# mrvollger/rustybam

Hardware: AMD Instinct MI355X
Metric: CIGAR-ops/s, liftover over 100 kb sliding windows (whole pass, inputs resident in HBM) (higher is better)
Workload: dtype u32

## Files before the change

### rustybam_amd/csrc/capi.hip

```cpp
#include <hip/hip_runtime.h>
#include <sys/mman.h>

#include <algorithm>
#include <cstdarg>
#include <cstdio>
#include <cstdlib>
#include <cstring>
#include <ctime>
#include <numeric>
#include <string>
#include <thread>
#include <vector>
#include <chrono>
#include <map>
#include <mutex>

#include "../../include/rustybam_amd.h"
#include "rb_lift.h"
#include "rb_trim.h"
#include "rb_launch.h"

#ifndef RB_SCAN_ROWS_MEAN_MAX
#define RB_SCAN_ROWS_MEAN_MAX 1536
#endif
// ... 676 lines not shown
    int rc = RB_OK;
    std::vector<uint32_t> slot_of(n_rec);
    for (uint64_t w = 0; w < n_rec; w++) slot_of[sched[w]] = (uint32_t)w;
    if (!rc) rc = upload_vec(ctx, sched, &pl->sched);
    if (!rc) rc = upload_vec(ctx, slot_of, &pl->slot_of);
    if (!rc) rc = upload_vec(ctx, ident, &pl->ident);
    if (!rc) rc = upload_vec(ctx, canon_pos, &pl->canon_pos);
    if (!rc) rc = upload_vec(ctx, g_st, &pl->w_st);
    if (!rc) rc = upload_vec(ctx, g_en, &pl->w_en);
    if (!rc) rc = upload_vec(ctx, g_orig, &pl->w_orig);
    if (!rc) rc = upload_vec(ctx, o_st, &pl->wo_st);
    if (!rc) rc = upload_vec(ctx, o_en, &pl->wo_en);
    if (!rc) rc = upload_vec(ctx, cw_off, &pl->cw_off);
    if (!rc) rc = upload_vec(ctx, mono, &pl->cw_mono);
    if (!rc && pl->n_tiles) rc = upload_vec(ctx, tiles, &pl->tiles);
    if (!rc && hipStreamSynchronize(ctx->stream) != hipSuccess) rc = fail(ctx, RB_E_HIP, "plan upload: %s", hipGetErrorString(hipGetLastError()));
    if (rc) {
        rb_plan_destroy(pl);
        return rc;
    }
    *out = pl;
    return RB_OK;
}
extern "C" void rb_plan_destroy(rb_plan *pl) {
    if (!pl) return;
    void *ptrs[] = {pl->sched, pl->slot_of, pl->ident, pl->canon_pos, pl->w_st, pl->w_en, pl->w_orig, pl->wo_st, pl->wo_en, pl->cw_off, pl->cw_mono, pl->tiles};
    for (void *q : ptrs)
        if (q) (void)rb_dev_free(pl->ctx, q);
    delete pl;
}

struct ws_layout {
    size_t hit_off, win_lo, block_sums, arena, pend_count, pend_list, jobs, gen_list, x_st, x_en, bp_tmp, bp_off, bp_cur, brk_rows, copy_count, copy_list, decl_count, decl_list, gen_cp, diag_stamps, fb_count, fb_list, starts_bad, total;
};
static bool rb_no_gen_cp() {
    static const bool v = getenv("RB_DEBUG_NO_GEN_CP") != nullptr;
    return v;
}
static ws_layout ws_of(uint64_t n_rec, uint64_t rows_cap, uint64_t n_ops) {
    ws_layout w;
    size_t o = 0;
    auto take = [&](size_t bytes) {
        size_t at = o;
        o += (bytes + 255) & ~(size_t)255;
        return at;
    };
    w.hit_off = take((n_rec + 2) * 8);
    w.win_lo = take((n_rec + 2) * 4);
    w.block_sums = take(rb_scan_block_sums_count(n_rec) * 8);
    w.arena = take((size_t)RB_MAX_ARENA * RB_ARENA_STRIDE * 8);
    w.pend_count = take(256);
    w.pend_list = take((n_rec + 1) * 4);
    w.jobs = take((n_rec + 1) * sizeof(rb_job));
    w.gen_list = take((rows_cap + 1) * 4);
    w.x_st = take((rows_cap + 1) * 8);
    w.x_en = take((rows_cap + 1) * 8);
    w.bp_tmp = take((rows_cap + 1) * 8);
    w.bp_off = take((n_rec + 1) * 8);
    w.bp_cur = take((size_t)RB_MAX_ARENA * 128);
    w.brk_rows = take((rows_cap + 1) * sizeof(rb_hit_row));
    w.copy_count = take(256);
    w.copy_list = take((rows_cap + 1) * 16);
    w.decl_count = take(256);
    w.decl_list = take((n_rec + 1) * 4);
    w.gen_cp = take(rb_no_gen_cp() ? 256 : (size_t)(n_ops / RB_GCP + n_rec + 2) * sizeof(uint4));
    w.diag_stamps = take((n_rec + 1) * 4);
    w.fb_count = take(256);
    w.fb_list = take((n_rec + 1) * 4);
    w.starts_bad = take(256);
    w.total = o;
    return w;
}
extern "C" size_t rb_plan_workspace_bytes(const rb_plan *plan, uint64_t rows_cap) {
    if (!plan) return 0;
    return ws_of(plan->n_rec, rows_cap, plan->n_ops).total;
}
extern "C" size_t rb_plan_diag_stamps_offset(const rb_plan *plan, uint64_t rows_cap) {
    if (!plan) return 0;
    return ws_of(plan->n_rec, rows_cap, plan->n_ops).diag_stamps;
}

static uint64_t slot_stride_of(uint64_t n_ops, uint64_t n_rec) { return ((n_ops + 31) & ~(uint64_t)31) + 32 * n_rec + 64; }
extern "C" uint64_t rb_plan_out_capacity(const rb_plan *plan, int for_break) {
    if (!plan) return 0;
    const uint64_t slots = for_break ? std::min<uint32_t>(2u, RB_MS) : std::min<uint32_t>(plan->depth, RB_MS);
    return slots * slot_stride_of(plan->n_ops, plan->n_rec) + plan->n_ops / 16 + 32 * plan->n_rec + (1u << 20);
}

static uint32_t pick_arenas(uint64_t n_rec) {
    uint64_t a = n_rec / 256;
    if (a < 1) a = 1;
    if (a > RB_MAX_ARENA) a = RB_MAX_ARENA;
    return (uint32_t)a;
}

static int lift_common(rb_ctx *ctx, const rb_plan *plan, const rb_batch_view *b, const rb_norm_row *norm, int policy,
                       void *workspace, rb_hit_row *rows, uint64_t rows_cap, uint32_t *out_ops, uint64_t out_cap,
                       rb_counters *counters, bool is_break, uint32_t max_size) {
    if (!ctx || !plan || !b || !norm || !workspace || !counters) return RB_E_INVALID;
    if (b->n_rec != plan->n_rec) return fail(ctx, RB_E_INVALID, "plan was built for %llu records, batch has %llu", (unsigned long long)plan->n_rec, (unsigned long long)b->n_rec);
// ... 51 lines not shown
    p.fused = (policy & RB_LIFT_FUSED_SCAN) ? 1 : 0;
    p.op_starts = (policy & RB_LIFT_OP_STARTS) ? 1 : 0;
    if (p.op_starts && p.fused) return fail(ctx, RB_E_INVALID, "RB_LIFT_OP_STARTS takes finished norm_rows: not together with RB_LIFT_FUSED_SCAN");
    if (p.op_starts && (policy & RB_LIFT_DESCRIPTORS)) return fail(ctx, RB_E_INVALID, "RB_LIFT_OP_STARTS with RB_LIFT_DESCRIPTORS: a descriptor indexes the record's ORIGINAL cigar, which a batch cut in place no longer is");
    if (p.op_starts && b->n_ops > plan->n_ops) return fail(ctx, RB_E_INVALID, "RB_LIFT_OP_STARTS: batch->n_ops exceeds the plan's op count (gather the batch first)");
    if (p.op_starts && b->n_rec) {
        unsigned long long *bad = (unsigned long long *)(ws + w.starts_bad), first_bad = 0;
        HIPCHK(ctx, rb_fill_async(bad, 0xFF, 8, ctx->stream));
        HIPCHK(ctx, rb_launch_starts_check(b->op_off, norm, b->n_rec, b->n_ops, bad, ctx->stream));
        HIPCHK(ctx, hipMemcpyAsync(&first_bad, bad, 8, hipMemcpyDeviceToHost, ctx->stream));
        HIPCHK(ctx, hipStreamSynchronize(ctx->stream));
        if (first_bad != ~0ull)
            return fail(ctx, RB_E_INVALID, "RB_LIFT_OP_STARTS: record %llu lies outside the batch's %llu ops (a pass moved it: gather the batch first)",
                        first_bad, (unsigned long long)b->n_ops);
    }
    p.norm_w = const_cast<rb_norm_row *>(norm);
    p.pend_list = (uint32_t *)(ws + w.pend_list);
    p.pend_count = (unsigned long long *)(ws + w.pend_count);
    const bool use_tiles = plan->n_tiles != 0 && ((policy >> 8) & 0xFFF) == 0;
    p.tile_first = use_tiles ? plan->tiles : nullptr;
    p.n_tiles = use_tiles ? plan->n_tiles : 0;
    p.fb_list = (uint32_t *)(ws + w.fb_list);
    p.fb_count = (unsigned long long *)(ws + w.fb_count);
    const uint32_t stream_end = use_tiles ? plan->stream_end : (uint32_t)b->n_rec;
    rb_scan_params sp;
    memset(&sp, 0, sizeof sp);
    if (p.fused) {
        sp.n_rec = b->n_rec;
        sp.ops = b->ops;
        sp.op_off = b->op_off;
        sp.t_st = b->t_st, sp.t_en = b->t_en, sp.q_st = b->q_st, sp.q_en = b->q_en;
        sp.strand = b->strand;
        sp.norm_rows = p.norm_w;
        HIPCHK(ctx, rb_fill_async(p.pend_count, 0, 8, ctx->stream));
        HIPCHK(ctx, rb_launch_peek_norm(&sp, ctx->stream));
    }
    p.counters = counters;
    p.policy = policy & 1;
    p.early_exit = (policy & RB_LIFT_EARLY_EXIT) ? 1 : 0;
    p.debug_skip = (policy >> 8) & 0xFFF;
    uint64_t *block_sums = (uint64_t *)(ws + w.block_sums);
    HIPCHK(ctx, rb_fill_async(counters, 0, sizeof(rb_counters), ctx->stream));
    HIPCHK(ctx, rb_fill_async(p.copy_count, 0, 8, ctx->stream));
    HIPCHK(ctx, rb_fill_async(p.arena_cur, 0, (size_t)RB_MAX_ARENA * RB_ARENA_STRIDE * 8, ctx->stream));
    if (b->n_rec == 0) return RB_OK;
    const bool one_walk = is_break && (policy & RB_BREAK_ONE_WALK) && !p.desc_mode;
    if (one_walk) {
        p.brk_mode = 1, p.brk_max = max_size;
        p.rows_final = rows;
        p.rows = (rb_hit_row *)(ws + w.brk_rows);
        p.brk_off = (uint64_t *)(ws + w.bp_off);
        p.brk_cursor = (unsigned long long *)(ws + w.bp_cur);
        p.brk_n_arena = pick_arenas(b->n_rec);
        p.brk_arena_cap = rows_cap / p.brk_n_arena;
        p.brk_decl_list = (uint32_t *)(ws + w.decl_list);
        p.brk_decl_count = (unsigned long long *)(ws + w.decl_count);
        HIPCHK(ctx, rb_fill_async(p.brk_decl_count, 0, 8, ctx->stream));
        HIPCHK(ctx, rb_fill_async(p.brk_cursor, 0, (size_t)RB_MAX_ARENA * 128, ctx->stream));
        HIPCHK(ctx, rb_fill_async(p.hit_off, 0, (size_t)(b->n_rec + 2) * 8, ctx->stream));
        HIPCHK(ctx, rb_fill_async(p.brk_off, 0xFF, (size_t)(b->n_rec + 1) * 8, ctx->stream));
        HIPCHK(ctx, rb_launch_make_jobs(&p, ctx->stream));
        const size_t slot1 = (size_t)(ctx->timed_calls % RB_TIMING_RING);
        if (ctx->timing) HIPCHK(ctx, hipEventRecord(ctx->ev_a[slot1], ctx->stream));
        p.wave0 = 0;
        p.wave_end = stream_end;
        HIPCHK(ctx, rb_launch_liftover_stream(&p, ctx->stream));
        if (use_tiles) {
            HIPCHK(ctx, rb_fill_async(p.fb_count, 0, 8, ctx->stream));
            HIPCHK(ctx, rb_launch_liftover_tiles(&p, ctx->stream));
            HIPCHK(ctx, rb_launch_liftover_stream_list(&p, ctx->stream));
        }
        if (p.fused) {
            sp.list = p.pend_list;
            sp.n_list = (const uint64_t *)p.pend_count;
            HIPCHK(ctx, rb_launch_scan_records(&sp, ctx->stream));
        }
        if (ctx->timing) {
            HIPCHK(ctx, hipEventRecord(ctx->ev_b[slot1], ctx->stream));
            ctx->timed_calls++;
        }
        rb_break_params bp;
        memset(&bp, 0, sizeof bp);
        bp.n_rec = b->n_rec, bp.ops = b->ops, bp.op_off = b->op_off, bp.norm = norm, bp.sched = plan->sched, bp.hit_off = p.hit_off;
        bp.x_st = (uint64_t *)(ws + w.x_st), bp.x_en = (uint64_t *)(ws + w.x_en);
        bp.rows_cap = rows_cap, bp.max_size = max_size;
        bp.list = p.brk_decl_list, bp.n_list = p.brk_decl_count;
        bp.fill = 0;
        HIPCHK(ctx, rb_launch_break_list_declined(&p, ctx->stream));
        HIPCHK(ctx, rb_launch_break_pieces(&bp, ctx->stream));
        HIPCHK(ctx, rb_launch_count_and_scan(&p, block_sums, false, ctx->stream));
        bp.fill = 1;
        HIPCHK(ctx, rb_launch_break_pieces(&bp, ctx->stream));
        HIPCHK(ctx, rb_launch_break_gather(&p, ctx->stream));
        rb_lift_params pg = p;
        pg.rows = rows, pg.x_st = bp.x_st, pg.x_en = bp.x_en;
        HIPCHK(ctx, rb_launch_break_declined(&pg, ctx->stream));
        return RB_OK;
    }
    if (is_break) {
        rb_break_params bp;
        memset(&bp, 0, sizeof bp);
        bp.n_rec = b->n_rec;
        bp.ops = b->ops;
        bp.op_off = b->op_off;
        bp.norm = norm;
        bp.sched = plan->sched;
        bp.hit_off = p.hit_off;
        bp.x_st = (uint64_t *)(ws + w.x_st);
        bp.x_en = (uint64_t *)(ws + w.x_en);
        bp.rows_cap = rows_cap;
        bp.max_size = max_size;
        bp.tmp = (uint2 *)(ws + w.bp_tmp);
        bp.tmp_off = (uint64_t *)(ws + w.bp_off);
        bp.tmp_cursor = (unsigned long long *)(ws + w.bp_cur);
        bp.n_arena = pick_arenas(b->n_rec);
        bp.arena_cap = rows_cap / bp.n_arena;
        HIPCHK(ctx, rb_fill_async(bp.tmp_cursor, 0, (size_t)RB_MAX_ARENA * 128, ctx->stream));
        bp.fill = 2, bp.redo_only = 0;
        HIPCHK(ctx, rb_launch_break_pieces(&bp, ctx->stream));
        HIPCHK(ctx, rb_launch_count_and_scan(&p, block_sums, false, ctx->stream));
        HIPCHK(ctx, rb_launch_break_place(&bp, ctx->stream));
        bp.fill = 1, bp.redo_only = 1;
        HIPCHK(ctx, rb_launch_break_pieces(&bp, ctx->stream));
        p.x_st = bp.x_st;
        p.x_en = bp.x_en;
    } else {
        HIPCHK(ctx, rb_launch_count_and_scan(&p, block_sums, true, ctx->stream));
    }
    HIPCHK(ctx, rb_launch_make_jobs(&p, ctx->stream));
    const size_t slot = (size_t)(ctx->timed_calls % RB_TIMING_RING);
    if (ctx->timing) HIPCHK(ctx, hipEventRecord(ctx->ev_a[slot], ctx->stream));
    p.wave0 = 0;
    p.wave_end = stream_end;
    HIPCHK(ctx, rb_launch_liftover_stream(&p, ctx->stream));
    if (use_tiles) {
        HIPCHK(ctx, rb_fill_async(p.fb_count, 0, 8, ctx->stream));
        HIPCHK(ctx, rb_launch_liftover_tiles(&p, ctx->stream));
        HIPCHK(ctx, rb_launch_liftover_stream_list(&p, ctx->stream));
    }
    if (p.fused) {
        sp.list = p.pend_list;
        sp.n_list = (const uint64_t *)p.pend_count;
        HIPCHK(ctx, rb_launch_scan_records(&sp, ctx->stream));
    }
    if (ctx->timing) {
        HIPCHK(ctx, hipEventRecord(ctx->ev_b[slot], ctx->stream));
        ctx->timed_calls++;
    }
    HIPCHK(ctx, rb_launch_liftover_tail(&p, ctx->stream));
    return RB_OK;
}

extern "C" int rb_dev_liftover(rb_ctx *ctx, const rb_plan *plan, const rb_batch_view *batch, const rb_norm_row *norm_rows,
                               int bsearch_policy, void *workspace, rb_hit_row *rows, uint64_t rows_cap, uint32_t *out_ops,
                               uint64_t out_cap, rb_counters *counters) {
    return lift_common(ctx, plan, batch, norm_rows, bsearch_policy, workspace, rows, rows_cap, out_ops, out_cap, counters, false, 0);
}
extern "C" int rb_dev_break(rb_ctx *ctx, const rb_plan *plan, const rb_batch_view *batch, const rb_norm_row *norm_rows,
                            uint32_t max_size, int bsearch_policy, void *workspace, rb_hit_row *rows, uint64_t rows_cap,
                            uint32_t *out_ops, uint64_t out_cap, rb_counters *counters) {
    return lift_common(ctx, plan, batch, norm_rows, bsearch_policy, workspace, rows, rows_cap, out_ops, out_cap, counters, true, max_size);
}

extern "C" int rb_dev_swap(rb_ctx *ctx, const rb_batch_view *b, uint32_t *out_ops) {
    if (!ctx || !b || !out_ops) return RB_E_INVALID;
    rb_swap_params p;
    p.n_rec = b->n_rec;
    p.ops = b->ops;
    p.op_off = b->op_off;
// ... 1091 lines not shown
```

### rustybam_amd/csrc/k_liftover.hip

```cpp
#include "rb_lift.h"
#include "rb_launch.h"
#include <type_traits>
#include <algorithm>

__global__ __launch_bounds__(256) void rb_k_count_hits(rb_lift_params p) {
    const uint64_t r = (uint64_t)blockIdx.x * blockDim.x + threadIdx.x;
    if (r >= p.n_rec) return;
    uint64_t cnt = 0;
    const rb_norm_row *nr = &p.norm[r];
    const uint32_t c = p.contig[r];
    if (nr->status == RB_ST_OK && c < p.n_contig) {
        const uint64_t ws = p.cw_off[c], we = p.cw_off[c + 1];
        const uint64_t t_st = nr->t_st, t_en = nr->t_en;
        if (p.cw_mono[c]) {
            const uint64_t lo = rb_lower_en_gt(p.w_en, ws, we, t_st);
            const uint64_t hi = rb_lower_st_ge(p.w_st, ws, we, t_en);
            cnt = hi > lo ? hi - lo : 0;
            p.win_lo[r] = (uint32_t)lo;
        } else {
            for (uint64_t i = ws; i < we; i++) cnt += (t_en > p.w_st[i] && t_st < p.w_en[i]) ? 1 : 0;
        }
    }
    p.hit_off[p.canon_pos[r]] = cnt;
}

#define RB_SCAN_PER_BLOCK 2048
__global__ __launch_bounds__(256) void rb_k_scan_partial(const uint64_t *v, uint64_t n, uint64_t *block_sums) {
    __shared__ uint64_t sh[4];
    const uint64_t base = (uint64_t)blockIdx.x * RB_SCAN_PER_BLOCK;
    uint64_t s = 0;
    for (int k = 0; k < RB_SCAN_PER_BLOCK / 256; k++) {
        uint64_t i = base + (uint64_t)k * 256 + threadIdx.x;
        if (i < n) s += v[i];
    }
    s = rb_wave_sum_u64(s);
    if ((threadIdx.x & 63) == 0) sh[threadIdx.x >> 6] = s;
    __syncthreads();
    if (threadIdx.x == 0) block_sums[blockIdx.x] = sh[0] + sh[1] + sh[2] + sh[3];
}
__global__ __launch_bounds__(256) void rb_k_scan_top(uint64_t *block_sums, uint64_t n_blocks) {
    __shared__ uint64_t sh[256];
    __shared__ uint64_t carry;
    if (threadIdx.x == 0) carry = 0;
    __syncthreads();
    for (uint64_t b = 0; b < n_blocks; b += 256) {
        uint64_t i = b + threadIdx.x;
        uint64_t x = i < n_blocks ? block_sums[i] : 0;
        sh[threadIdx.x] = x;
        __syncthreads();
        for (int off = 1; off < 256; off <<= 1) {
            uint64_t y = threadIdx.x >= (unsigned)off ? sh[threadIdx.x - off] : 0;
            __syncthreads();
            sh[threadIdx.x] += y;
            __syncthreads();
        }
        uint64_t incl = sh[threadIdx.x];
// ... 37 lines not shown
}

__global__ __launch_bounds__(256) void rb_k_make_jobs(rb_lift_params p) {
    const uint64_t r64 = (uint64_t)blockIdx.x * blockDim.x + threadIdx.x;
    if (r64 >= p.n_rec) return;
    const uint32_t r = (uint32_t)r64;
    const uint64_t w = p.slot_of[r];
    const rb_norm_row *nr = &p.norm[r];
    rb_job j;
    j.r = r;
    j.n = nr->n_ops;
    j.rec0 = p.op_off[r] + nr->first_op;
    j.t_st = nr->t_st, j.t_en = nr->t_en, j.q_st = nr->q_st, j.q_en = nr->q_en;
    const uint64_t k = p.canon_pos[r];
    const bool brk = p.brk_mode != 0;
    const uint64_t h0 = brk ? 0ull : p.hit_off[k], nh = brk ? 1ull : p.hit_off[k + 1] - h0;
    const bool explicit_w = brk || p.x_st != nullptr;
    const uint32_t cg = p.contig[r];
    const bool mono = explicit_w || (cg < p.n_contig && p.cw_mono[cg] != 0);
    uint32_t f = 0;
    const bool provisional = (nr->flags & RB_F_PROVISIONAL) != 0;
    if (nr->status == RB_ST_OK && (nh != 0 || provisional)) {
        if (h0 + nh > p.rows_cap) f |= RB_JOB_ROWS_OVERFLOW;
        else f |= RB_JOB_VALID;
    }
    if ((nr->flags & RB_F_REGULAR) || (provisional && !(nr->flags & RB_F_ENDS_NOT_MATCH))) f |= RB_JOB_REGULAR;
    if (p.strand[r] == (uint8_t)'-') f |= RB_JOB_MINUS;
    if (mono) f |= RB_JOB_MONO;
    j.flags = f;
    j.h0 = (uint32_t)h0;
    j.nh = (uint32_t)nh;
    j.lo = (explicit_w || !mono || !(f & RB_JOB_VALID) || nh == 0) ? 0u : p.win_lo[r];
    p.jobs[w] = j;
}

#define RB_RING_BASE 80
#define RB_RING_TOP_N 95
#define RB_SPILL_ROOM 0
#define RB_WPE 5, 6
#include "rb_stream.h"
#define RB_STREAM_KERNEL(NAME, BRK, DIAG, ROOM)                                                                                   \
    __global__ __launch_bounds__(256) __attribute__((amdgpu_waves_per_eu(RB_WPE), amdgpu_num_vgpr(RB_RING_BASE - (ROOM)))) void NAME(rb_lift_params p_) { \
        (void)p_;                                 \
        rb_stream_record<BRK, DIAG>();                                                                                            \
    }
RB_STREAM_KERNEL(rb_k_liftover_stream, false, false, RB_SPILL_ROOM)
RB_STREAM_KERNEL(rb_k_liftover_stream_brk, true, false, RB_SPILL_ROOM)
RB_STREAM_KERNEL(rb_k_liftover_stream_diag, false, true, 4)

__global__ __launch_bounds__(256) void rb_k_copy_clips(rb_lift_params p) {
    const uint64_t n_copy = *p.copy_count;
    const int lane = rb_lane();
    for (uint64_t e = (uint64_t)blockIdx.x * 4u + (threadIdx.x >> 6); e < n_copy; e += (uint64_t)gridDim.x * 4u) {
        const uint4 d = p.copy_list[e];
        rb_hit_row *row = &p.rows[d.x];
        const uint32_t rec = row->rec, n = row->out_n;
        const uint32_t *src = p.ops + p.op_off[rec] + p.norm[rec].first_op + d.y;
        const uint32_t padded = (n + 3u) & ~3u;
        const uint32_t arena = (uint32_t)(e % p.n_arena);
        unsigned long long b0 = 0;
        if (lane == 0) b0 = atomicAdd(&p.arena_cur[(uint64_t)arena * RB_ARENA_STRIDE], (unsigned long long)padded);
        b0 = rb_first64(b0);
        if (b0 + padded > p.arena_size) {
            if (lane == 0) p.counters->overflow = 1;
            continue;
        }
// ... 820 lines not shown
            row->rec = r;
            row->win = (uint32_t)j;
            row->flags = RB_HIT_GENERIC;
            const unsigned long long g = atomicAdd((unsigned long long *)&p.counters->n_generic, 1ull);
            p.gen_list[g] = (uint32_t)h;
        }
    }
}
extern "C" hipError_t rb_launch_break_declined(const rb_lift_params *p, hipStream_t stream) {
    if (p->n_rec == 0) return hipSuccess;
    hipLaunchKernelGGL(rb_k_break_declined_rows, dim3((unsigned)std::min<uint64_t>((p->n_rec + 255) / 256, 256)), dim3(256), 0, stream, *p);
    if (p->gen_cp) hipLaunchKernelGGL(rb_k_generic_checkpoints, dim3(2048), dim3(256), 0, stream, *p);
    hipLaunchKernelGGL(rb_k_generic_jobs, dim3(1024), dim3(256), 0, stream, *p);
    hipLaunchKernelGGL(rb_k_liftover_generic_wave, dim3(2048), dim3(256), 0, stream, *p);
    hipLaunchKernelGGL(rb_k_finish, dim3(1), dim3(64), 0, stream, *p);
    return hipGetLastError();
}
extern "C" hipError_t rb_launch_count_and_scan(const rb_lift_params *p, uint64_t *block_sums, bool do_count, hipStream_t stream) {
    if (p->n_rec == 0) return hipSuccess;
    if (do_count) {
        const unsigned blocks = (unsigned)((p->n_rec + 255) / 256);
        hipLaunchKernelGGL(rb_k_count_hits, dim3(blocks), dim3(256), 0, stream, *p);
    }
    return rb_launch_exclusive_scan(p->hit_off, p->n_rec, block_sums, &p->counters->n_hits, stream);
}
extern "C" hipError_t rb_launch_exclusive_scan(uint64_t *v, uint64_t n, uint64_t *block_sums, uint64_t *total_out, hipStream_t stream) {
    if (n == 0) return hipSuccess;
    const uint64_t nb = (n + RB_SCAN_PER_BLOCK - 1) / RB_SCAN_PER_BLOCK;
    hipLaunchKernelGGL(rb_k_scan_partial, dim3((unsigned)nb), dim3(256), 0, stream, (const uint64_t *)v, n, block_sums);
    hipLaunchKernelGGL(rb_k_scan_top, dim3(1), dim3(256), 0, stream, block_sums, nb);
    hipLaunchKernelGGL(rb_k_scan_apply, dim3((unsigned)nb), dim3(256), 0, stream, v, n, (const uint64_t *)block_sums, total_out);
    return hipGetLastError();
}
extern "C" hipError_t rb_launch_make_jobs(const rb_lift_params *p, hipStream_t stream) {
    if (p->n_rec == 0) return hipSuccess;
    hipLaunchKernelGGL(rb_k_make_jobs, dim3((unsigned)((p->n_rec + 255) / 256)), dim3(256), 0, stream, *p);
    return hipGetLastError();
}

extern "C" hipError_t rb_launch_liftover_stream(const rb_lift_params *p, hipStream_t stream) {
    if (p->n_rec == 0 || p->wave_end <= p->wave0) return hipSuccess;
    const unsigned blocks = (unsigned)(((uint64_t)(p->wave_end - p->wave0) + 3) / 4);
    if (p->debug_skip) {
        if (!p->brk_mode) {
            hipLaunchKernelGGL(rb_k_liftover_stream_diag, dim3(blocks), dim3(256), 0, stream, *p);
            return hipGetLastError();
        }
    }
    if (p->brk_mode) hipLaunchKernelGGL(rb_k_liftover_stream_brk, dim3(blocks), dim3(256), 0, stream, *p);
    else hipLaunchKernelGGL(rb_k_liftover_stream, dim3(blocks), dim3(256), 0, stream, *p);
    return hipGetLastError();
}
extern "C" hipError_t rb_launch_liftover_tail(const rb_lift_params *p, hipStream_t stream) {
    if (p->n_rec == 0) return hipSuccess;
    hipLaunchKernelGGL(rb_k_copy_clips, dim3(2048), dim3(256), 0, stream, *p);
    if (p->gen_cp) hipLaunchKernelGGL(rb_k_generic_checkpoints, dim3(2048), dim3(256), 0, stream, *p);
    hipLaunchKernelGGL(rb_k_generic_jobs, dim3(1024), dim3(256), 0, stream, *p);
    hipLaunchKernelGGL(rb_k_liftover_generic_wave, dim3(2048), dim3(256), 0, stream, *p);
    hipLaunchKernelGGL(rb_k_finish, dim3(1), dim3(64), 0, stream, *p);
    return hipGetLastError();
}

extern "C" size_t rb_scan_block_sums_count(uint64_t n_rec) { return (size_t)((n_rec + RB_SCAN_PER_BLOCK - 1) / RB_SCAN_PER_BLOCK + 2); }
```

### rustybam_amd/csrc/k_records.hip

```cpp
#include "rb_device.h"
#include "rb_launch.h"
#include <algorithm>
#include <type_traits>

struct rb_strip {
    uint32_t lead, trail;
    uint64_t dR, dQ;
    uint64_t t_st, t_en, q_st, q_en;
};
__device__ __forceinline__ rb_strip rb_strip_ends(const uint32_t *ops, uint64_t n, uint64_t t_st, uint64_t t_en, uint64_t q_st, uint64_t q_en,
                                                  bool minus) {
    rb_strip o;
    uint64_t lead = 0, rm_st_t = 0, rm_st_q = 0;
    uint32_t prev = RB_NULL_OP;
    o.dR = o.dQ = 0;
    while (lead < n) {
        uint32_t opc, len;
        const uint32_t words = rb_op_fwd(ops, n, lead, &opc, &len);
        if (!rb_in(RB_INDEL_MASK, opc)) break;
        if (opc == RB_OP_D) {
            rm_st_t += len;
            rm_st_q += 1;
            o.dR += len;
        } else {
            rm_st_q += len;
            o.dQ += len;
        }
        if (prev != RB_NULL_OP && prev != opc) {
            rm_st_t += 1;
            rm_st_q -= 1;
        }
        prev = opc;
        lead += words;
    }
    uint64_t trail = 0, rm_en_t = 0, rm_en_q = 0;
    while (trail < n) {
        uint32_t opc, len;
        const uint32_t words = rb_op_bwd(ops, n - 1 - trail, &opc, &len);
        if (!rb_in(RB_INDEL_MASK, opc)) break;
        if (opc == RB_OP_D) {
            rm_en_t += len;
            if (lead + trail < n) o.dR += len;
        } else {
            rm_en_q += len;
            if (lead + trail < n) o.dQ += len;
        }
        trail += words;
    }
    o.lead = (uint32_t)lead;
    o.trail = (uint32_t)trail;
    o.t_st = t_st + rm_st_t, o.t_en = t_en - rm_en_t;
    if (minus) {
        const uint64_t t = rm_st_q;
        rm_st_q = rm_en_q;
        rm_en_q = t;
    }
    o.q_st = q_st + rm_st_q, o.q_en = q_en - rm_en_q;
    return o;
}

__global__ __launch_bounds__(256) void rb_k_peek_norm(rb_scan_params p) {
    const uint64_t r = (uint64_t)blockIdx.x * blockDim.x + threadIdx.x;
    if (r >= p.n_rec) return;
    const uint64_t o0 = p.op_off[r], n = p.op_off[r + 1] - o0;
    rb_norm_row w;
    w.t_st = w.t_en = w.q_st = w.q_en = 0;
    w.first_op = w.n_ops = w.lead_ops = w.trail_ops = w.nmatch = w.aln_len = 0;
    w.flags = RB_F_PROVISIONAL;
    uint32_t st = RB_ST_OK;
    if (n == 0) {
        st = RB_ST_PANIC_EMPTY_CIGAR;
    } else {
        const bool minus = p.strand && p.strand[r] == (uint8_t)'-';
        const rb_strip sp = rb_strip_ends(p.ops + o0, n, p.t_st[r], p.t_en[r], p.q_st[r], p.q_en[r], minus);
        w.lead_ops = sp.lead;
        w.trail_ops = sp.trail;
        if (sp.lead || sp.trail) w.flags |= RB_F_STRIPPED;
        if ((uint64_t)sp.lead + sp.trail > n) {
            st = RB_ST_PANIC_ALL_INDEL;
        } else {
            w.t_st = sp.t_st, w.t_en = sp.t_en, w.q_st = sp.q_st, w.q_en = sp.q_en;
            w.first_op = sp.lead;
            w.n_ops = (uint32_t)(n - sp.lead - sp.trail);
            const uint32_t fo = rb_opc(p.ops[o0 + sp.lead]), lo_ = rb_opc(p.ops[o0 + n - 1 - sp.trail]);
            if (fo > 8u || lo_ > 8u || !rb_in(RB_MATCH_MASK, fo) || !rb_in(RB_MATCH_MASK, lo_)) w.flags |= RB_F_ENDS_NOT_MATCH;
        }
    }
    if (st != RB_ST_OK) w.flags &= ~(uint32_t)RB_F_PROVISIONAL;
    w.status = st;
    p.norm_rows[r] = w;
}

__device__ __forceinline__ void rb_scan_finish(const rb_scan_params &p, const uint64_t r, const uint64_t (&L)[9], const uint32_t ins_events,
                                               const uint32_t del_events, const uint32_t bad, const uint64_t o0, const uint64_t o1, const uint64_t t_st,
                                               const uint64_t t_en, const uint64_t q_st, const uint64_t q_en, const bool minus) {
    const uint64_t n = o1 - o0;
    const uint64_t R = L[RB_OP_M] + L[RB_OP_D] + L[RB_OP_N] + L[RB_OP_EQ] + L[RB_OP_X];
    const uint64_t Q = L[RB_OP_M] + L[RB_OP_I] + L[RB_OP_S] + L[RB_OP_EQ] + L[RB_OP_X];
    const uint64_t M = L[RB_OP_M] + L[RB_OP_EQ] + L[RB_OP_X];
    uint64_t U = 0;
#pragma unroll
    for (int t = 0; t < 9; t++) U += L[t];
    uint32_t flags = 0;
    if (bad == 0 && U <= 0xFFFFFFFFull) flags |= RB_F_REGULAR;
    if (L[RB_OP_M] != 0) flags |= RB_F_HAS_M;

    if (p.reduce_rows) {
        rb_reduce_row w;
        w.t_bases = R;
        w.q_bases = Q;
        w.nmatch = (uint32_t)M;
        w.aln_len = (uint32_t)U;
        w.equal = (uint32_t)L[RB_OP_EQ];
        w.diff = (uint32_t)(L[RB_OP_X] + L[RB_OP_M]);
        w.ins = (uint32_t)L[RB_OP_I];
        w.del = (uint32_t)L[RB_OP_D];
        w.matches = (uint32_t)L[RB_OP_M];
        w.ins_events = ins_events;
        w.del_events = del_events;
        const float num = 100.0f * (float)w.equal;
        w.id_by_all = num / (float)(uint32_t)(w.equal + w.diff + w.del + w.ins);
        w.id_by_events = num / (float)(uint32_t)(w.equal + w.diff + w.del_events + w.ins_events);
        w.id_by_matches = num / (float)(uint32_t)(w.equal + w.diff);
// ... 241 lines not shown
                if (any_edge) step(std::true_type{});
                else step(std::false_type{});
            }
        }
    }
    uint64_t L[9];
    auto sum40 = [&](unsigned long long v) -> uint64_t {
        const uint32_t s_lo = rb_row_sum((uint32_t)v & 0xFFFFFu), s_hi = rb_row_sum((uint32_t)(v >> 20) & 0xFFFFFu);
        return (uint64_t)s_lo + ((uint64_t)s_hi << 20);
    };
#pragma unroll
    for (int t = 0; t < 9; t++)
        if (t != RB_OP_H && t != RB_OP_P) L[t] = sum40(hist[t][lane]);
    {
        const unsigned long long h = hist[RB_OP_H][lane], q = hist[RB_OP_P][lane];
        const uint32_t s_lo = rb_row_sum(((uint32_t)h & 0xFFFFFu) + ((uint32_t)q & 0xFFFFFu));
        const uint32_t s_hi = rb_row_sum(((uint32_t)(h >> 20) & 0xFFFFFu) + ((uint32_t)(q >> 20) & 0xFFFFFu));
        L[RB_OP_H] = (uint64_t)s_lo + ((uint64_t)s_hi << 20);
        L[RB_OP_P] = 0;
    }
    const uint32_t ins_events = rb_row_sum((uint32_t)(hist[RB_OP_I][lane] >> RB_LEN_BITS));
    const uint32_t del_events = rb_row_sum((uint32_t)(hist[RB_OP_D][lane] >> RB_LEN_BITS));
    uint32_t bad = (v_reg != 0xFFFFFFFFu ? 1u : 0u) | (v_minlen == 0u ? 2u : 0u) | (v_adj == 0u ? 4u : 0u) | v_big;
    bad = (rb_row_ballot((bad & 1u) != 0u, gbase) ? 1u : 0u) | (rb_row_ballot((bad & 2u) != 0u, gbase) ? 2u : 0u) |
          (rb_row_ballot((bad & 4u) != 0u, gbase) ? 4u : 0u) | (rb_row_ballot((bad & 8u) != 0u, gbase) ? 8u : 0u);
    if (take && gl == 0u) rb_scan_finish(p, r, L, ins_events, del_events, bad, o0, o1, t_st, t_en, q_st, q_en, minus);
}

extern "C" hipError_t rb_launch_peek_norm(const rb_scan_params *p, hipStream_t stream) {
    if (p->n_rec == 0) return hipSuccess;
    hipLaunchKernelGGL(rb_k_peek_norm, dim3((unsigned)((p->n_rec + 255) / 256)), dim3(256), 0, stream, *p);
    return hipGetLastError();
}
extern "C" hipError_t rb_launch_scan_records(const rb_scan_params *p, hipStream_t stream) {
    if (p->n_rec == 0) return hipSuccess;
    const uint64_t blocks = p->list ? std::min<uint64_t>((p->n_rec + 3) / 4, 1024) : (p->n_rec + 3) / 4;
    hipLaunchKernelGGL(rb_k_scan_records, dim3((unsigned)blocks), dim3(256), 0, stream, *p);
    return hipGetLastError();
}
extern "C" hipError_t rb_launch_scan_rows(const rb_scan_params *p, void *long_buf, hipStream_t stream) {
    if (p->n_rec == 0) return hipSuccess;
    unsigned long long *n_long = (unsigned long long *)long_buf;
    uint32_t *long_list = (uint32_t *)((char *)long_buf + 256);
    hipLaunchKernelGGL(rb_k_scan_rows, dim3((unsigned)((p->n_rec + 15) / 16)), dim3(256), 0, stream, *p, n_long, long_list);
    rb_scan_params q = *p;
    q.list = long_list, q.n_list = (const uint64_t *)n_long;
    const uint64_t blocks = std::min<uint64_t>((p->n_rec + 3) / 4, 8192);
    hipLaunchKernelGGL(rb_k_scan_records, dim3((unsigned)blocks), dim3(256), 0, stream, q);
    return hipGetLastError();
}
```

### rustybam_amd/csrc/rb_launch.h

```cpp
#pragma once
#include <hip/hip_runtime.h>
#include <stdint.h>

#include "../../include/rustybam_amd.h"

struct rb_lift_params;
struct rb_trim_params;
struct nf_read;
struct nf_tdesc;

struct rb_scan_params {
    uint64_t n_rec;
    const uint32_t *ops;
    const uint64_t *op_off;
    const uint64_t *t_st, *t_en, *q_st, *q_en;
    const uint8_t *strand;
    rb_reduce_row *reduce_rows;
    rb_norm_row *norm_rows;
    const uint32_t *list;
    const uint64_t *n_list;
};
extern "C" hipError_t rb_launch_scan_records(const rb_scan_params *p, hipStream_t stream);
extern "C" hipError_t rb_launch_scan_rows(const rb_scan_params *p, void *long_buf, hipStream_t stream);
extern "C" hipError_t rb_launch_peek_norm(const rb_scan_params *p, hipStream_t stream);

extern "C" hipError_t rb_launch_count_and_scan(const rb_lift_params *p, uint64_t *block_sums, bool do_count, hipStream_t stream);
extern "C" hipError_t rb_launch_exclusive_scan(uint64_t *v, uint64_t n, uint64_t *block_sums, uint64_t *total_out, hipStream_t stream);
extern "C" size_t rb_scan_block_sums_count(uint64_t n_rec);
extern "C" hipError_t rb_launch_make_jobs(const rb_lift_params *p, hipStream_t stream);
extern "C" hipError_t rb_launch_liftover_stream(const rb_lift_params *p, hipStream_t stream);
extern "C" hipError_t rb_launch_liftover_tail(const rb_lift_params *p, hipStream_t stream);
extern "C" hipError_t rb_launch_liftover_stream_list(const rb_lift_params *p, hipStream_t stream);
extern "C" hipError_t rb_launch_liftover_tiles(const rb_lift_params *p, hipStream_t stream);
extern "C" uint32_t rb_tile_max_ops(void);
extern "C" uint32_t rb_tile_max_records(void);
extern "C" hipError_t rb_launch_break_gather(const rb_lift_params *p, hipStream_t stream);
extern "C" hipError_t rb_launch_break_declined(const rb_lift_params *p, hipStream_t stream);
extern "C" hipError_t rb_launch_break_list_declined(const rb_lift_params *p, hipStream_t stream);

struct rb_break_params {
    uint64_t n_rec;
    const uint32_t *ops;
    const uint64_t *op_off;
    const rb_norm_row *norm;
    const uint32_t *sched;
    uint64_t *hit_off;
    uint64_t *x_st, *x_en;
    uint64_t rows_cap;
    uint32_t max_size;
    int fill;
    int redo_only;
    uint2 *tmp;
    uint64_t *tmp_off;
    unsigned long long *tmp_cursor;
    uint32_t n_arena;
    uint64_t arena_cap;
    const uint32_t *list;
    const unsigned long long *n_list;
};
struct rb_swap_params {
    uint64_t n_rec;
    const uint32_t *ops;
// ... 148 lines not shown
```

### rustybam_amd/csrc/rb_lift.h

```cpp
#pragma once
#include "rb_device.h"
#include <cstdlib>


#define RB_HMAX 32
#define RB_LDS_PER_HIT 6
#define RB_ARENA_STRIDE 16
#define RB_MS 2

struct __attribute__((aligned(64))) rb_job {
    uint64_t rec0;
    uint32_t n;
    uint32_t r;
    uint32_t h0;
    uint32_t flags;
    uint32_t nh;
    uint32_t lo;
    uint64_t t_st, t_en, q_st, q_en;
};
enum { RB_JOB_VALID = 1, RB_JOB_REGULAR = 2, RB_JOB_MINUS = 4, RB_JOB_MONO = 8, RB_JOB_ROWS_OVERFLOW = 16 };

struct rb_lift_params {
    uint64_t n_rec;
    const uint32_t *ops;
    const uint64_t *op_off;
    const uint32_t *contig;
    const uint8_t *strand;
    const rb_norm_row *norm;
    const uint32_t *sched;
    const uint32_t *slot_of;
    const uint32_t *canon_pos;
    const uint64_t *w_st, *w_en;
    const uint32_t *w_orig;
    const uint64_t *wo_st, *wo_en;
    const uint64_t *cw_off;
    const uint8_t *cw_mono;
    uint32_t n_contig;
    const uint64_t *x_st, *x_en;
    uint64_t *hit_off;
    uint32_t *win_lo;
    rb_hit_row *rows;
    uint64_t rows_cap;
    uint32_t *out_ops;
    uint64_t out_cap;
    unsigned long long *arena_cur;
    uint64_t arena_size;
    uint32_t n_arena;
    uint32_t *gen_list;
    rb_counters *counters;
    int policy;
    int early_exit;
    int desc_mode;
    uint64_t arena_origin;
// ... 29 lines not shown
    unsigned long long *fb_count;
    int op_starts;
};
#define RB_GCP 64u
struct __attribute__((aligned(64))) rb_gja {
    uint64_t ops_off;
    uint64_t t_st, t_en, q_st, q_en;
    uint64_t wst, wen;
    uint32_t n;
    uint32_t k2;
};

typedef const __attribute__((address_space(4))) rb_lift_params *rb_kparams;
__device__ __forceinline__ rb_kparams rb_kp_here(rb_kparams q) {
    asm volatile("" : "+s"(q));
    return q;
}

__device__ __forceinline__ uint64_t rb_lower_en_gt(const uint64_t *w_en, uint64_t lo, uint64_t hi, uint64_t t_st) {
    while (lo < hi) {
        uint64_t mid = lo + ((hi - lo) >> 1);
        if (w_en[mid] > t_st) hi = mid; else lo = mid + 1;
    }
    return lo;
}
__device__ __forceinline__ uint64_t rb_lower_st_ge(const uint64_t *w_st, uint64_t lo, uint64_t hi, uint64_t t_en) {
    while (lo < hi) {
        uint64_t mid = lo + ((hi - lo) >> 1);
        if (w_st[mid] >= t_en) hi = mid; else lo = mid + 1;
    }
    return lo;
}

enum { RB_S_UNRES = 0, RB_S_OK = 1, RB_S_NONE = 2, RB_S_DEFER = 3 };

__device__ __forceinline__ int rb_ffs64(unsigned long long m) { return __ffsll((long long)m) - 1; }

__device__ inline void rb_defer_record(rb_kparams kp, uint32_t r, const rb_norm_row *nr, uint64_t h0, uint64_t nh,
                                bool explicit_w, bool mono, uint64_t ws, uint64_t we, int lane) {
    asm volatile("" : "+v"(lane));
    const rb_kparams q_ = rb_kp_here(kp);
    struct { const uint64_t *w_st, *w_en; const uint32_t *w_orig; rb_hit_row *rows; uint64_t rows_cap; uint32_t *gen_list; rb_counters *counters; } p =
        {q_->w_st, q_->w_en, q_->w_orig, q_->rows, q_->rows_cap, q_->gen_list, q_->counters};
    if (explicit_w || mono) {
        uint64_t lo = 0;
        if (!explicit_w) lo = rb_lower_en_gt(p.w_en, ws, we, nr->t_st);
        for (uint64_t j = lane; j < nh; j += 64) {
            const uint64_t h = h0 + j;
            if (h < p.rows_cap) {
                rb_hit_row *row = &p.rows[h];
                row->rec = r;
                row->win = explicit_w ? (uint32_t)j : p.w_orig[lo + j];
                row->flags = RB_HIT_GENERIC;
                const unsigned long long g = atomicAdd((unsigned long long *)&p.counters->n_generic, 1ull);
                p.gen_list[g] = (uint32_t)h;
            }
        }
    } else {
        uint64_t done = 0;
        for (uint64_t b = ws; b < we; b += 64) {
            const uint64_t i = b + lane;
            const bool hit = i < we && nr->t_en > p.w_st[i] && nr->t_st < p.w_en[i];
            const unsigned long long ball = __ballot(hit);
            if (hit) {
                const uint64_t j = done + __popcll(ball & ((1ull << lane) - 1ull));
                const uint64_t h = h0 + j;
// ... 196 lines not shown
```

Measured before the change: 531.2 billion.

## Fuse lift setup: peek+count+job build in one kernel, scan patches jobs

Merges the normalisation peek, hit counting and job construction into one setup kernel. A new scan-apply kernel writes the exclusive prefix and patches each job's h0/flags/nh/lo in place. This removes separate make_jobs and count launches, and it collapses several small memsets into one contiguous fill by regrouping the workspace layout. The fused kernel keeps intermediate state in job flag bits, which adds coupling between kernels. The win_lo array is reused as a slot index.

```diff
diff --git a/rustybam_amd/csrc/capi.hip b/rustybam_amd/csrc/capi.hip
--- a/rustybam_amd/csrc/capi.hip
+++ b/rustybam_amd/csrc/capi.hip
@@ -732,6 +732,7 @@
 
 struct ws_layout {
     size_t hit_off, win_lo, block_sums, arena, pend_count, pend_list, jobs, gen_list, x_st, x_en, bp_tmp, bp_off, bp_cur, brk_rows, copy_count, copy_list, decl_count, decl_list, gen_cp, diag_stamps, fb_count, fb_list, starts_bad, total;
+    size_t zero_lift, zero_break;
 };
 static bool rb_no_gen_cp() {
     static const bool v = getenv("RB_DEBUG_NO_GEN_CP") != nullptr;
@@ -750,6 +751,12 @@
     w.block_sums = take(rb_scan_block_sums_count(n_rec) * 8);
     w.arena = take((size_t)RB_MAX_ARENA * RB_ARENA_STRIDE * 8);
     w.pend_count = take(256);
+    w.copy_count = take(256);
+    w.fb_count = take(256);
+    w.zero_lift = o - w.arena;
+    w.decl_count = take(256);
+    w.bp_cur = take((size_t)RB_MAX_ARENA * 128);
+    w.zero_break = o - w.arena;
     w.pend_list = take((n_rec + 1) * 4);
     w.jobs = take((n_rec + 1) * sizeof(rb_job));
     w.gen_list = take((rows_cap + 1) * 4);
@@ -757,15 +764,11 @@
     w.x_en = take((rows_cap + 1) * 8);
     w.bp_tmp = take((rows_cap + 1) * 8);
     w.bp_off = take((n_rec + 1) * 8);
-    w.bp_cur = take((size_t)RB_MAX_ARENA * 128);
     w.brk_rows = take((rows_cap + 1) * sizeof(rb_hit_row));
-    w.copy_count = take(256);
     w.copy_list = take((rows_cap + 1) * 16);
-    w.decl_count = take(256);
     w.decl_list = take((n_rec + 1) * 4);
     w.gen_cp = take(rb_no_gen_cp() ? 256 : (size_t)(n_ops / RB_GCP + n_rec + 2) * sizeof(uint4));
     w.diag_stamps = take((n_rec + 1) * 4);
-    w.fb_count = take(256);
     w.fb_list = take((n_rec + 1) * 4);
     w.starts_bad = take(256);
     w.total = o;
@@ -883,8 +886,6 @@
         sp.t_st = b->t_st, sp.t_en = b->t_en, sp.q_st = b->q_st, sp.q_en = b->q_en;
         sp.strand = b->strand;
         sp.norm_rows = p.norm_w;
-        HIPCHK(ctx, rb_fill_async(p.pend_count, 0, 8, ctx->stream));
-        HIPCHK(ctx, rb_launch_peek_norm(&sp, ctx->stream));
     }
     p.counters = counters;
     p.policy = policy & 1;
@@ -892,9 +893,9 @@
     p.debug_skip = (policy >> 8) & 0xFFF;
     uint64_t *block_sums = (uint64_t *)(ws + w.block_sums);
     HIPCHK(ctx, rb_fill_async(counters, 0, sizeof(rb_counters), ctx->stream));
-    HIPCHK(ctx, rb_fill_async(p.copy_count, 0, 8, ctx->stream));
-    HIPCHK(ctx, rb_fill_async(p.arena_cur, 0, (size_t)RB_MAX_ARENA * RB_ARENA_STRIDE * 8, ctx->stream));
+    HIPCHK(ctx, rb_fill_async(ws + w.arena, 0, is_break ? w.zero_break : w.zero_lift, ctx->stream));
     if (b->n_rec == 0) return RB_OK;
+    if (p.fused && is_break) HIPCHK(ctx, rb_launch_peek_norm(&sp, ctx->stream));
     const bool one_walk = is_break && (policy & RB_BREAK_ONE_WALK) && !p.desc_mode;
     if (one_walk) {
         p.brk_mode = 1, p.brk_max = max_size;
@@ -906,8 +907,6 @@
         p.brk_arena_cap = rows_cap / p.brk_n_arena;
         p.brk_decl_list = (uint32_t *)(ws + w.decl_list);
         p.brk_decl_count = (unsigned long long *)(ws + w.decl_count);
-        HIPCHK(ctx, rb_fill_async(p.brk_decl_count, 0, 8, ctx->stream));
-        HIPCHK(ctx, rb_fill_async(p.brk_cursor, 0, (size_t)RB_MAX_ARENA * 128, ctx->stream));
         HIPCHK(ctx, rb_fill_async(p.hit_off, 0, (size_t)(b->n_rec + 2) * 8, ctx->stream));
         HIPCHK(ctx, rb_fill_async(p.brk_off, 0xFF, (size_t)(b->n_rec + 1) * 8, ctx->stream));
         HIPCHK(ctx, rb_launch_make_jobs(&p, ctx->stream));
@@ -917,7 +916,6 @@
         p.wave_end = stream_end;
         HIPCHK(ctx, rb_launch_liftover_stream(&p, ctx->stream));
         if (use_tiles) {
-            HIPCHK(ctx, rb_fill_async(p.fb_count, 0, 8, ctx->stream));
             HIPCHK(ctx, rb_launch_liftover_tiles(&p, ctx->stream));
             HIPCHK(ctx, rb_launch_liftover_stream_list(&p, ctx->stream));
         }
@@ -966,7 +964,6 @@
         bp.tmp_cursor = (unsigned long long *)(ws + w.bp_cur);
         bp.n_arena = pick_arenas(b->n_rec);
         bp.arena_cap = rows_cap / bp.n_arena;
-        HIPCHK(ctx, rb_fill_async(bp.tmp_cursor, 0, (size_t)RB_MAX_ARENA * 128, ctx->stream));
         bp.fill = 2, bp.redo_only = 0;
         HIPCHK(ctx, rb_launch_break_pieces(&bp, ctx->stream));
         HIPCHK(ctx, rb_launch_count_and_scan(&p, block_sums, false, ctx->stream));
@@ -975,17 +972,17 @@
         HIPCHK(ctx, rb_launch_break_pieces(&bp, ctx->stream));
         p.x_st = bp.x_st;
         p.x_en = bp.x_en;
+        HIPCHK(ctx, rb_launch_make_jobs(&p, ctx->stream));
     } else {
-        HIPCHK(ctx, rb_launch_count_and_scan(&p, block_sums, true, ctx->stream));
-    }
-    HIPCHK(ctx, rb_launch_make_jobs(&p, ctx->stream));
+        HIPCHK(ctx, rb_launch_setup_records(&p, p.fused ? &sp : nullptr, ctx->stream));
+        HIPCHK(ctx, rb_launch_scan_jobs(&p, block_sums, ctx->stream));
+    }
     const size_t slot = (size_t)(ctx->timed_calls % RB_TIMING_RING);
     if (ctx->timing) HIPCHK(ctx, hipEventRecord(ctx->ev_a[slot], ctx->stream));
     p.wave0 = 0;
     p.wave_end = stream_end;
     HIPCHK(ctx, rb_launch_liftover_stream(&p, ctx->stream));
     if (use_tiles) {
-        HIPCHK(ctx, rb_fill_async(p.fb_count, 0, 8, ctx->stream));
         HIPCHK(ctx, rb_launch_liftover_tiles(&p, ctx->stream));
         HIPCHK(ctx, rb_launch_liftover_stream_list(&p, ctx->stream));
     }
diff --git a/rustybam_amd/csrc/k_liftover.hip b/rustybam_amd/csrc/k_liftover.hip
--- a/rustybam_amd/csrc/k_liftover.hip
+++ b/rustybam_amd/csrc/k_liftover.hip
@@ -2,26 +2,15 @@
 #include "rb_launch.h"
 #include <type_traits>
 #include <algorithm>
+#include <cstddef>
 
 __global__ __launch_bounds__(256) void rb_k_count_hits(rb_lift_params p) {
     const uint64_t r = (uint64_t)blockIdx.x * blockDim.x + threadIdx.x;
     if (r >= p.n_rec) return;
-    uint64_t cnt = 0;
     const rb_norm_row *nr = &p.norm[r];
-    const uint32_t c = p.contig[r];
-    if (nr->status == RB_ST_OK && c < p.n_contig) {
-        const uint64_t ws = p.cw_off[c], we = p.cw_off[c + 1];
-        const uint64_t t_st = nr->t_st, t_en = nr->t_en;
-        if (p.cw_mono[c]) {
-            const uint64_t lo = rb_lower_en_gt(p.w_en, ws, we, t_st);
-            const uint64_t hi = rb_lower_st_ge(p.w_st, ws, we, t_en);
-            cnt = hi > lo ? hi - lo : 0;
-            p.win_lo[r] = (uint32_t)lo;
-        } else {
-            for (uint64_t i = ws; i < we; i++) cnt += (t_en > p.w_st[i] && t_st < p.w_en[i]) ? 1 : 0;
-        }
-    }
-    p.hit_off[p.canon_pos[r]] = cnt;
+    const rb_rec_hits h = rb_record_hits(p, nr->status, p.contig[r], nr->t_st, nr->t_en);
+    if (h.has_lo) p.win_lo[r] = h.lo;
+    p.hit_off[p.canon_pos[r]] = h.cnt;
 }
 
 #define RB_SCAN_PER_BLOCK 2048
@@ -125,6 +114,57 @@
     j.nh = (uint32_t)nh;
     j.lo = (explicit_w || !mono || !(f & RB_JOB_VALID) || nh == 0) ? 0u : p.win_lo[r];
     p.jobs[w] = j;
+}
+
+static_assert(offsetof(rb_job, h0) == 16 && offsetof(rb_job, flags) == 20 && offsetof(rb_job, nh) == 24 && offsetof(rb_job, lo) == 28,
+              "rb_k_jobs_hits updates {h0, flags, nh, lo} as the job's second 16 bytes");
+__global__ __launch_bounds__(256) void rb_k_jobs_hits(rb_lift_params p, const uint64_t *block_sums) {
+    __shared__ uint64_t sh[256];
+    constexpr int PER = RB_SCAN_PER_BLOCK / 256;
+    const uint64_t n = p.n_rec;
+    uint64_t *v = p.hit_off;
+    const uint64_t i0 = (uint64_t)blockIdx.x * RB_SCAN_PER_BLOCK + (uint64_t)threadIdx.x * PER;
+    uint64_t x[PER];
+    uint4 *slot[PER];
+    uint4 d[PER];
+    uint64_t s = 0;
+#pragma unroll
+    for (int k = 0; k < PER; k++) {
+        x[k] = (i0 + k < n) ? v[i0 + k] : 0;
+        s += x[k];
+    }
+#pragma unroll
+    for (int k = 0; k < PER; k++) {
+        slot[k] = reinterpret_cast<uint4 *>(&p.jobs[(i0 + k < n) ? p.win_lo[i0 + k] : 0u]) + 1;
+        d[k] = (i0 + k < n) ? *slot[k] : make_uint4(0u, 0u, 0u, 0u);
+    }
+    sh[threadIdx.x] = s;
+    __syncthreads();
+    for (int off = 1; off < 256; off <<= 1) {
+        uint64_t y = threadIdx.x >= (unsigned)off ? sh[threadIdx.x - off] : 0;
+        __syncthreads();
+        sh[threadIdx.x] += y;
+        __syncthreads();
+    }
+    uint64_t run = block_sums[blockIdx.x] + sh[threadIdx.x] - s;
+#pragma unroll
+    for (int k = 0; k < PER; k++) {
+        if (i0 + k < n) {
+            const uint64_t h0 = run, nh = x[k];
+            v[i0 + k] = h0;
+            uint32_t f = d[k].y & ~(uint32_t)(RB_JOB_SETUP_OK | RB_JOB_SETUP_PROVISIONAL);
+            if ((d[k].y & RB_JOB_SETUP_OK) && (nh != 0 || (d[k].y & RB_JOB_SETUP_PROVISIONAL)))
+                f |= h0 + nh > p.rows_cap ? RB_JOB_ROWS_OVERFLOW : RB_JOB_VALID;
+            const uint32_t lo = (!(f & RB_JOB_MONO) || !(f & RB_JOB_VALID) || nh == 0) ? 0u : d[k].w;
+            *slot[k] = make_uint4((uint32_t)h0, f, (uint32_t)nh, lo);
+        }
+        run += x[k];
+    }
+    if (blockIdx.x == gridDim.x - 1 && threadIdx.x == 255) {
+        const uint64_t total = block_sums[gridDim.x];
+        v[n] = total;
+        p.counters->n_hits = total;
+    }
 }
 
 #define RB_RING_BASE 80
@@ -1011,6 +1051,14 @@
     hipLaunchKernelGGL(rb_k_scan_apply, dim3((unsigned)nb), dim3(256), 0, stream, v, n, (const uint64_t *)block_sums, total_out);
     return hipGetLastError();
 }
+extern "C" hipError_t rb_launch_scan_jobs(const rb_lift_params *p, uint64_t *block_sums, hipStream_t stream) {
+    if (p->n_rec == 0) return hipSuccess;
+    const uint64_t nb = (p->n_rec + RB_SCAN_PER_BLOCK - 1) / RB_SCAN_PER_BLOCK;
+    hipLaunchKernelGGL(rb_k_scan_partial, dim3((unsigned)nb), dim3(256), 0, stream, (const uint64_t *)p->hit_off, p->n_rec, block_sums);
+    hipLaunchKernelGGL(rb_k_scan_top, dim3(1), dim3(256), 0, stream, block_sums, nb);
+    hipLaunchKernelGGL(rb_k_jobs_hits, dim3((unsigned)nb), dim3(256), 0, stream, *p, (const uint64_t *)block_sums);
+    return hipGetLastError();
+}
 extern "C" hipError_t rb_launch_make_jobs(const rb_lift_params *p, hipStream_t stream) {
     if (p->n_rec == 0) return hipSuccess;
     hipLaunchKernelGGL(rb_k_make_jobs, dim3((unsigned)((p->n_rec + 255) / 256)), dim3(256), 0, stream, *p);
diff --git a/rustybam_amd/csrc/k_records.hip b/rustybam_amd/csrc/k_records.hip
--- a/rustybam_amd/csrc/k_records.hip
+++ b/rustybam_amd/csrc/k_records.hip
@@ -1,4 +1,5 @@
 #include "rb_device.h"
+#include "rb_lift.h"
 #include "rb_launch.h"
 #include <algorithm>
 #include <type_traits>
@@ -59,9 +60,7 @@
     return o;
 }
 
-__global__ __launch_bounds__(256) void rb_k_peek_norm(rb_scan_params p) {
-    const uint64_t r = (uint64_t)blockIdx.x * blockDim.x + threadIdx.x;
-    if (r >= p.n_rec) return;
+__device__ __forceinline__ rb_norm_row rb_peek_row(const rb_scan_params &p, const uint64_t r) {
     const uint64_t o0 = p.op_off[r], n = p.op_off[r + 1] - o0;
     rb_norm_row w;
     w.t_st = w.t_en = w.q_st = w.q_en = 0;
@@ -88,7 +87,49 @@
     }
     if (st != RB_ST_OK) w.flags &= ~(uint32_t)RB_F_PROVISIONAL;
     w.status = st;
-    p.norm_rows[r] = w;
+    return w;
+}
+__global__ __launch_bounds__(256) void rb_k_peek_norm(rb_scan_params p) {
+    const uint64_t r = (uint64_t)blockIdx.x * blockDim.x + threadIdx.x;
+    if (r >= p.n_rec) return;
+    p.norm_rows[r] = rb_peek_row(p, r);
+}
+
+template <bool PROV>
+__global__ __launch_bounds__(256) void rb_k_setup_records(rb_lift_params p, rb_scan_params sp) {
+    const uint64_t r64 = (uint64_t)blockIdx.x * blockDim.x + threadIdx.x;
+    if (r64 >= p.n_rec) return;
+    const uint32_t r = (uint32_t)r64;
+    rb_norm_row w;
+    if (PROV) {
+        w = rb_peek_row(sp, r64);
+        sp.norm_rows[r] = w;
+    } else {
+        w = p.norm[r];
+    }
+    const uint32_t cg = p.contig[r];
+    const rb_rec_hits h = rb_record_hits(p, w.status, cg, w.t_st, w.t_en);
+    const uint32_t slot = p.slot_of[r];
+    const uint64_t k = p.canon_pos[r];
+    p.hit_off[k] = h.cnt;
+    p.win_lo[k] = slot;
+    rb_job j;
+    j.r = r;
+    j.n = w.n_ops;
+    j.rec0 = p.op_off[r] + w.first_op;
+    j.t_st = w.t_st, j.t_en = w.t_en, j.q_st = w.q_st, j.q_en = w.q_en;
+    const bool provisional = (w.flags & RB_F_PROVISIONAL) != 0;
+    uint32_t f = 0;
+    if ((w.flags & RB_F_REGULAR) || (provisional && !(w.flags & RB_F_ENDS_NOT_MATCH))) f |= RB_JOB_REGULAR;
+    if (p.strand[r] == (uint8_t)'-') f |= RB_JOB_MINUS;
+    if (cg < p.n_contig && p.cw_mono[cg] != 0) f |= RB_JOB_MONO;
+    if (w.status == RB_ST_OK) f |= RB_JOB_SETUP_OK;
+    if (provisional) f |= RB_JOB_SETUP_PROVISIONAL;
+    j.flags = f;
+    j.h0 = 0;
+    j.nh = 0;
+    j.lo = h.has_lo ? h.lo : 0u;
+    p.jobs[slot] = j;
 }
 
 __device__ __forceinline__ void rb_scan_finish(const rb_scan_params &p, const uint64_t r, const uint64_t (&L)[9], const uint32_t ins_events,
@@ -396,6 +437,13 @@
     hipLaunchKernelGGL(rb_k_peek_norm, dim3((unsigned)((p->n_rec + 255) / 256)), dim3(256), 0, stream, *p);
     return hipGetLastError();
 }
+extern "C" hipError_t rb_launch_setup_records(const rb_lift_params *p, const rb_scan_params *sp, hipStream_t stream) {
+    if (p->n_rec == 0) return hipSuccess;
+    const dim3 grid((unsigned)((p->n_rec + 255) / 256));
+    if (sp) hipLaunchKernelGGL(rb_k_setup_records<true>, grid, dim3(256), 0, stream, *p, *sp);
+    else hipLaunchKernelGGL(rb_k_setup_records<false>, grid, dim3(256), 0, stream, *p, rb_scan_params{});
+    return hipGetLastError();
+}
 extern "C" hipError_t rb_launch_scan_records(const rb_scan_params *p, hipStream_t stream) {
     if (p->n_rec == 0) return hipSuccess;
     const uint64_t blocks = p->list ? std::min<uint64_t>((p->n_rec + 3) / 4, 1024) : (p->n_rec + 3) / 4;
diff --git a/rustybam_amd/csrc/rb_launch.h b/rustybam_amd/csrc/rb_launch.h
--- a/rustybam_amd/csrc/rb_launch.h
+++ b/rustybam_amd/csrc/rb_launch.h
@@ -23,11 +23,13 @@
 extern "C" hipError_t rb_launch_scan_records(const rb_scan_params *p, hipStream_t stream);
 extern "C" hipError_t rb_launch_scan_rows(const rb_scan_params *p, void *long_buf, hipStream_t stream);
 extern "C" hipError_t rb_launch_peek_norm(const rb_scan_params *p, hipStream_t stream);
+extern "C" hipError_t rb_launch_setup_records(const rb_lift_params *p, const rb_scan_params *sp, hipStream_t stream);
 
 extern "C" hipError_t rb_launch_count_and_scan(const rb_lift_params *p, uint64_t *block_sums, bool do_count, hipStream_t stream);
 extern "C" hipError_t rb_launch_exclusive_scan(uint64_t *v, uint64_t n, uint64_t *block_sums, uint64_t *total_out, hipStream_t stream);
 extern "C" size_t rb_scan_block_sums_count(uint64_t n_rec);
 extern "C" hipError_t rb_launch_make_jobs(const rb_lift_params *p, hipStream_t stream);
+extern "C" hipError_t rb_launch_scan_jobs(const rb_lift_params *p, uint64_t *block_sums, hipStream_t stream);
 extern "C" hipError_t rb_launch_liftover_stream(const rb_lift_params *p, hipStream_t stream);
 extern "C" hipError_t rb_launch_liftover_tail(const rb_lift_params *p, hipStream_t stream);
 extern "C" hipError_t rb_launch_liftover_stream_list(const rb_lift_params *p, hipStream_t stream);
diff --git a/rustybam_amd/csrc/rb_lift.h b/rustybam_amd/csrc/rb_lift.h
--- a/rustybam_amd/csrc/rb_lift.h
+++ b/rustybam_amd/csrc/rb_lift.h
@@ -19,6 +19,7 @@
     uint64_t t_st, t_en, q_st, q_en;
 };
 enum { RB_JOB_VALID = 1, RB_JOB_REGULAR = 2, RB_JOB_MINUS = 4, RB_JOB_MONO = 8, RB_JOB_ROWS_OVERFLOW = 16 };
+enum : uint32_t { RB_JOB_SETUP_OK = 1u << 30, RB_JOB_SETUP_PROVISIONAL = 1u << 31 };
 
 struct rb_lift_params {
     uint64_t n_rec;
@@ -114,6 +115,28 @@
     return lo;
 }
 
+struct rb_rec_hits {
+    uint64_t cnt;
+    uint32_t lo;
+    bool has_lo;
+};
+__device__ __forceinline__ rb_rec_hits rb_record_hits(const rb_lift_params &p, uint32_t status, uint32_t c, uint64_t t_st, uint64_t t_en) {
+    rb_rec_hits o;
+    o.cnt = 0, o.lo = 0, o.has_lo = false;
+    if (status == RB_ST_OK && c < p.n_contig) {
+        const uint64_t ws = p.cw_off[c], we = p.cw_off[c + 1];
+        if (p.cw_mono[c]) {
+            const uint64_t lo = rb_lower_en_gt(p.w_en, ws, we, t_st);
+            const uint64_t hi = rb_lower_st_ge(p.w_st, ws, we, t_en);
+            o.cnt = hi > lo ? hi - lo : 0;
+            o.lo = (uint32_t)lo, o.has_lo = true;
+        } else {
+            for (uint64_t i = ws; i < we; i++) o.cnt += (t_en > p.w_st[i] && t_st < p.w_en[i]) ? 1 : 0;
+        }
+    }
+    return o;
+}
+
 enum { RB_S_UNRES = 0, RB_S_OK = 1, RB_S_NONE = 2, RB_S_DEFER = 3 };
 
 __device__ __forceinline__ int rb_ffs64(unsigned long long m) { return __ffsll((long long)m) - 1; }
```

Measured after the change: 532.1 billion, median of 2. Within noise of the previous version (+0.2%).
